# EmbodiedVision/diffsdfsim

Measured on AMD Instinct MI355X. Metric: sim steps/sec (fwd+bwd), 1024 batched 3D scenes x 8 SDF bodies, higher is better.
Workload: dtype f64

## Files before the change

### diffsdfsim_amd/csrc/contact_geom.h

```cpp
#pragma once
#include "geom.h"

namespace dss {
#if DSS_ALL_SHAPES
inline namespace shapes_all {
#else
inline namespace shapes_lean {
#endif

template <class T> struct BodyG {
    T q[4], pos[3];
    Shape<T> shape;
};

template <class T> __host__ __device__ inline double lap_probe(const Shape<T> &s, const T *p, double phi0, double h)
{
    Shape<double> sd;
    sd.type = s.type;
    for (int i = 0; i < 3; ++i) { sd.prm[i] = val(s.prm[i]); sd.hd[i] = val(s.hd[i]); }
    sd.scale = val(s.scale);
#if DSS_ALL_SHAPES
    sd.hr = val(s.hr);
    sd.lin = nullptr;
    sd.grid = s.grid;
    for (int i = 0; i < 3; ++i) sd.gn[i] = s.gn[i];
#endif
    double acc = 0.0, pt[3] = {val(p[0]), val(p[1]), val(p[2])}, g[3];
    for (int i = 0; i < 3; ++i) {
        double a, b, save = pt[i];
        pt[i] = save + h; query_sdf(sd, pt, a, g, false);
        pt[i] = save - h; query_sdf(sd, pt, b, g, false);
        pt[i] = save;
        acc += a - 2.0 * phi0 + b;
    }
    return acc;
}

template <class T>
__host__ __device__ inline void contact_head(const BodyG<T> &b1, const T tri[3][3], const double abc[3], T *cp1, T *n1, T &d1,
                                             T *p1)
{
    for (int i = 0; i < 3; ++i) cp1[i] = tri[0][i] * abc[0] + tri[1][i] * abc[1] + tri[2][i] * abc[2];
#if DSS_ALL_SHAPES
    if (b1.shape.type == SHAPE_IGR) {
        igr_lin(b1.shape, 0, cp1, d1, n1);
        for (int i = 0; i < 3; ++i) cp1[i] = cp1[i] - d1 * n1[i];
        igr_lin(b1.shape, 1, cp1, d1, n1);
        quat_apply(b1.q, cp1, p1);
        return;
    }
#endif
    query_sdf(b1.shape, cp1, d1, n1, true);
    for (int i = 0; i < 3; ++i) cp1[i] = cp1[i] - d1 * n1[i];
    query_sdf(b1.shape, cp1, d1, n1, true);
    quat_apply(b1.q, cp1, p1);
}
template <class T>
__host__ __device__ inline void contact_tail(const BodyG<T> &b1, const BodyG<T> &b2, const T *cp1, const T *n1, const T &d1,
                                             const T *p1, double lap_h, T *n, T *p2, T &pen, int *stable_io, bool detach_b2 = false)
{
    T cpw[3], rel[3], cp2[3], d2, n2[3], t[3];
    for (int i = 0; i < 3; ++i) { cpw[i] = p1[i] + b1.pos[i]; rel[i] = cpw[i] - b2.pos[i]; }
    quat_apply_inv(b2.q, rel, cp2);
    if (detach_b2) for (int i = 0; i < 3; ++i) cp2[i] = T(val(cp2[i]));
#if DSS_ALL_SHAPES
    if (b2.shape.type == SHAPE_IGR) igr_lin(b2.shape, 0, cp2, d2, n2);
    else
#endif
    query_sdf(b2.shape, cp2, d2, n2, true);
    bool stable;
    if (stable_io && *stable_io >= 0) stable = *stable_io != 0;
    else {
        const double l1 = lap_probe(b1.shape, cp1, val(d1), lap_h), l2 = lap_probe(b2.shape, cp2, val(d2), lap_h);
        stable = fabs(l2) < fabs(l1);
        if (stable_io) *stable_io = stable ? 1 : 0;
    }
    if (stable) {
        quat_apply(b2.q, n2, n);
    } else {
        quat_apply(b1.q, n1, t);
        for (int i = 0; i < 3; ++i) n[i] = -t[i];
    }
    for (int i = 0; i < 3; ++i) t[i] = cp2[i] - d2 * n2[i];
    quat_apply(b2.q, t, p2);
    pen = -d2;
}
template <class T>
__host__ __device__ inline void contact_from_bary(const BodyG<T> &b1, const BodyG<T> &b2, const T tri[3][3],
                                                  const double abc[3], double lap_h, T *n, T *p1, T *p2, T &pen,
                                                  int *stable_io = nullptr, bool detach_b2 = false)
{
    T cp1[3], n1[3], d1;
    contact_head(b1, tri, abc, cp1, n1, d1, p1);
    contact_tail(b1, b2, cp1, n1, d1, p1, lap_h, n, p2, pen, stable_io, detach_b2);
}

template <class T> __host__ __device__ inline T toc_D(const T *in)
{
    const T h = in[0], hc = in[1];
    const T *p1 = in + 2, *p2 = in + 5, *n = in + 8, *V1 = in + 11, *V2 = in + 17, *q1 = in + 23, *x1 = in + 27,
            *q2 = in + 30, *x2 = in + 34, *a1 = in + 37, *a2 = in + 40;
    T R1[9], R2[9], r1[9], r2[9], R10[9], R20[9], w[3], pos1[3], pos2[3];
    for (int i = 0; i < 3; ++i) { pos1[i] = x1[i] - hc * V1[3 + i]; pos2[i] = x2[i] - hc * V2[3 + i]; }
    for (int i = 0; i < 3; ++i) w[i] = -hc * V1[i];
    so3_exp(w, r1);
    for (int i = 0; i < 3; ++i) w[i] = -hc * V2[i];
    so3_exp(w, r2);
    quat_to_mat(q1, R1);
    quat_to_mat(q2, R2);
    for (int a = 0; a < 3; ++a)
        for (int b = 0; b < 3; ++b) {
            R10[3 * a + b] = r1[3 * a] * R1[b] + r1[3 * a + 1] * R1[3 + b] + r1[3 * a + 2] * R1[6 + b];
            R20[3 * a + b] = r2[3 * a] * R2[b] + r2[3 * a + 1] * R2[3 + b] + r2[3 * a + 2] * R2[6 + b];
        }
    T cs1[3], cs2[3], ns2[3];
    for (int i = 0; i < 3; ++i) {
        cs1[i] = R10[i] * p1[0] + R10[3 + i] * p1[1] + R10[6 + i] * p1[2];
        cs2[i] = R20[i] * p2[0] + R20[3 + i] * p2[1] + R20[6 + i] * p2[2];
        ns2[i] = R20[i] * n[0] + R20[3 + i] * n[1] + R20[6 + i] * n[2];
    }
    T dRi[9], dRj[9], Rih[9], Rjh[9];
    for (int i = 0; i < 3; ++i) w[i] = h * V1[i];
    so3_exp(w, dRi);
    for (int i = 0; i < 3; ++i) w[i] = h * V2[i];
    so3_exp(w, dRj);
    for (int a = 0; a < 3; ++a)
        for (int b = 0; b < 3; ++b) {
            Rih[3 * a + b] = dRi[3 * a] * R10[b] + dRi[3 * a + 1] * R10[3 + b] + dRi[3 * a + 2] * R10[6 + b];
            Rjh[3 * a + b] = dRj[3 * a] * R20[b] + dRj[3 * a + 1] * R20[3 + b] + dRj[3 * a + 2] * R20[6 + b];
        }
    T ciw[3], rel[3], D = T(0.0);
    for (int i = 0; i < 3; ++i) {
        const T pih = pos1[i] + h * V1[3 + i] + 0.5 * a1[i] * h * h, pjh = pos2[i] + h * V2[3 + i] + 0.5 * a2[i] * h * h;
        ciw[i] = Rih[3 * i] * cs1[0] + Rih[3 * i + 1] * cs1[1] + Rih[3 * i + 2] * cs1[2] + pih;
        rel[i] = ciw[i] - pjh;
    }
    for (int i = 0; i < 3; ++i) {
        const T cij = Rjh[i] * rel[0] + Rjh[3 + i] * rel[1] + Rjh[6 + i] * rel[2];
        D = D + ns2[i] * (cs2[i] - cij);
    }
    return D;
}

template <class T> __host__ __device__ inline void friction_dirs(const T *n, int nd, T D[][3])
{
    int am = 0;
    for (int i = 1; i < 3; ++i) if (fabs(val(n[i])) < fabs(val(n[am]))) am = i;
    T e[3] = {T(am == 0 ? 1.0 : 0.0), T(am == 1 ? 1.0 : 0.0), T(am == 2 ? 1.0 : 0.0)}, t[3];
    cross(e, n, t);
    normalize(t, D[0]);
    cross(D[0], n, t);
    normalize(t, D[1]);
    if (nd == 4) {
        for (int i = 0; i < 3; ++i) t[i] = D[0][i] + D[1][i];
        normalize(t, D[2]);
        cross(D[2], n, t);
        normalize(t, D[3]);
    }
}

}
}
```

### diffsdfsim_amd/csrc/narrowphase.hip

```cpp
#ifndef DSS_ALL_SHAPES
#define DSS_ALL_SHAPES 0
#endif
#if !DSS_ALL_SHAPES
#define DSS_STAMPS np
#endif

#include "launchers.h"
#include "np_common.h"

namespace {
constexpr int NP_WAVES = 3;
constexpr int OV_RUN = 256;
constexpr int OV_NT = 256;
__global__ void __launch_bounds__(OV_NT) overlap_kernel(DssWorld W)
{
    __shared__ unsigned char s_ok[64 * 63 / 2];
    __shared__ unsigned char s_big[64];
    const int nb = W.nb, nup = nb * (nb - 1) / 2, np = npairs_of(nb);
    const int sc = blockIdx.x, tid = threadIdx.x, lane = tid & 63, wv = tid >> 6;
    if (!W.active[sc]) return;
    const bool few = (long)W.B * np <= 256L * NP_WAVES;
    if (tid < nb) {
        const int nf = W.mesh_nf[W.mesh_id[(size_t)sc * nb + tid]];
        s_big[tid] = nf > WAVE_ITEM_MAX_FACES || (few && nf > 2048);
    }
#if DSS_ALL_SHAPES
    __shared__ unsigned char s_igr[64];
    if (tid < nb) s_igr[tid] = W.shape_type[(size_t)sc * nb + tid] == DSS_SHAPE_IGR;
#endif
    for (int up = wv; up < nup; up += OV_NT / 64) {
        int i = 0, rem = up;
        while (rem >= nb - 1 - i) { rem -= nb - 1 - i; ++i; }
        const int j = i + 1 + rem;
        int ok = !W.no_contact[i * nb + j];
        if (ok) {
            BodyD A, Bd;
            load_body(W, sc, i, A);
            load_body(W, sc, j, Bd);
            for (int dir = 0; dir < 2 && ok; ++dir) {
                const BodyD &src = dir ? Bd : A, &dst = dir ? A : Bd;
                const double s = dst.g.shape.scale;
                Region reg;
                region_of(src.g, dst.g, 1e-9, reg);
                const double *vbox = W.vch_box + (size_t)W.mesh_vch_off[src.mesh] * 6;
                const int nch = (src.nv + OV_RUN - 1) / OV_RUN;
                int found = 0;
                for (int cb0 = 0; cb0 < nch && !found; cb0 += 64) {
                    const int ch = cb0 + lane;
                    unsigned long long m = __ballot(ch < nch && box_hits(reg, vbox + (size_t)ch * 6));
                    while (m && !found) {
                        const int b = __ffsll((long long)m) - 1;
                        m &= m - 1;
                        int hit = 0;
#pragma unroll
                        for (int sub = 0; sub < OV_RUN / 64; ++sub) {
                            const int v = (cb0 + b) * OV_RUN + sub * 64 + lane;
                            if (v < src.nv) {
                                double p[3];
                                to_frame(src.g, dst.g, W.verts + (size_t)(src.voff + v) * 3, p);
                                hit |= (-s <= p[0] && p[0] <= s && -s <= p[1] && p[1] <= s && -s <= p[2] && p[2] <= s);
                            }
                        }
                        found = __ballot(hit) != 0ull;
                    }
                }
                ok = found;
            }
        }
        if (lane == 0) {
            s_ok[up] = (unsigned char)ok;
            W.ovl[((size_t)sc * nb + i) * nb + j] = ok;
            if (!ok) {
                W.pc_count[(size_t)sc * np + i * (nb - 1) + (j - 1)] = 0;
                W.pc_count[(size_t)sc * np + j * (nb - 1) + i] = 0;
            }
        }
    }
    __syncthreads();
    if (tid == 0) {
        int cnt[2] = {0, 0};
#if DSS_ALL_SHAPES
        int nig = 0;
        for (int up = 0, i = 0, j = 1; up < nup; ++up) {
            if (s_ok[up] && (s_igr[i] || s_igr[j])) nig += 2;
            if (++j == nb) { ++i; j = i + 1; }
        }
        if (nig) {
            int at = atomicAdd(W.n_pairs + 6, nig);
            for (int up = 0, i = 0, j = 1; up < nup; ++up) {
                if (s_ok[up] && (s_igr[i] || s_igr[j])) {
                    s_ok[up] = 0;
                    if (W.igr_list && at + 2 <= W.igr_items_cap) {
                        W.igr_list[at++] = sc * np + i * (nb - 1) + (j - 1);
                        W.igr_list[at++] = sc * np + j * (nb - 1) + i;
                    } else atomicOr(W.overflow + sc, 32);
                }
                if (++j == nb) { ++i; j = i + 1; }
            }
        }
#endif
        for (int up = 0, i = 0, j = 1; up < nup; ++up) {
            if (s_ok[up]) { ++cnt[s_big[i] ? 0 : 1]; ++cnt[s_big[j] ? 0 : 1]; }
            if (++j == nb) { ++i; j = i + 1; }
        }
        const int cap = W.B * np;
        const unsigned long long old = atomicAdd(reinterpret_cast<unsigned long long *>(W.n_pairs),
                                                 (unsigned long long)(unsigned)cnt[0] | ((unsigned long long)(unsigned)cnt[1] << 32));
        int at[2] = {(int)(old & 0xffffffffull), (int)(old >> 32)};
        for (int up = 0, i = 0, j = 1; up < nup; ++up) {
            if (s_ok[up]) {
                const int li = s_big[i] ? 0 : 1, lj = s_big[j] ? 0 : 1;
                W.pair_list[(size_t)li * cap + at[li]++] = sc * np + i * (nb - 1) + (j - 1);
                W.pair_list[(size_t)lj * cap + at[lj]++] = sc * np + j * (nb - 1) + i;
            }
            if (++j == nb) { ++i; j = i + 1; }
        }
    }
}

template <class G> __device__ int narrow_pair(const DssWorld &W, ScratchT<G> &S, int item, int slot_id)
{
    STAMP(0);
    item = dss_uniform(item); slot_id = dss_uniform(slot_id);
    const int np = npairs_of(W.nb);
    const int sc = item / np, dp = item % np, tid = G::tid();
    int a, b;
    pair_of(dp, W.nb, a, b);
    int *pc_count = W.pc_count + (size_t)sc * np + dp;
    BodyD A, Bd;
    load_body(W, sc, a, A);
    load_body(W, sc, b, Bd);
    const int MC = W.max_cand;
    int *__restrict__ cface = W.cand_face + (size_t)slot_id * 2 * MC, *__restrict__ kface = cface + MC;
    int *__restrict__ cstate = W.cand_state + (size_t)slot_id * MC;
    double *__restrict__ cb = W.cand_buf + (size_t)slot_id * DSS_CAND_FIELDS * MC;
    const double *__restrict__ m_verts = W.verts, *__restrict__ m_fcent = W.fcent;
    const int *__restrict__ m_faces = W.faces;
#define CB(f, k) cb[(size_t)(f) * MC + (k)]
    const double sB = Bd.g.shape.scale;

    double Ra[9], Rb[9], R12[9], t12[3];
    quat_to_mat(A.g.q, Ra);
    quat_to_mat(Bd.g.q, Rb);
    for (int i = 0; i < 3; ++i) {
        for (int j = 0; j < 3; ++j) R12[3 * i + j] = Rb[i] * Ra[j] + Rb[3 + i] * Ra[3 + j] + Rb[6 + i] * Ra[6 + j];
        t12[i] = Rb[i] * (A.g.pos[0] - Bd.g.pos[0]) + Rb[3 + i] * (A.g.pos[1] - Bd.g.pos[1]) + Rb[6 + i] * (A.g.pos[2] - Bd.g.pos[2]);
    }

    int ncand = 0, over = 0;
    Region reg;
    region_of(A.g, Bd.g, 1e-9, reg);
    const double *fbox = W.fch_box + (size_t)W.mesh_fch_off[A.mesh] * 6;
    constexpr int RUN = 256;
    const int nch = (A.nf + RUN - 1) / RUN, lane = tid & 63, wv = tid >> 6;
    auto cull_face = [&](const double *c) -> int {
        double cb2[3];
        for (int i = 0; i < 3; ++i) cb2[i] = R12[3 * i] * c[0] + R12[3 * i + 1] * c[1] + R12[3 * i + 2] * c[2] + t12[i];
        const double lim = sB + 1e-9 * (1.0 + sB);
        return fabs(cb2[0]) <= lim && fabs(cb2[1]) <= lim && fabs(cb2[2]) <= lim;
    };
    auto load_tri = [&](int f, double tri[3][3]) {
        const int *fv = m_faces + (size_t)(A.foff + f) * 3;
        for (int k = 0; k < 3; ++k) {
            const double *vp = m_verts + (size_t)(A.voff + fv[k]) * 3;
            for (int i = 0; i < 3; ++i) tri[k][i] = vp[i];
        }
    };
    auto test_tri = [&](double tri[3][3], double pqr[3][3]) -> int {
        double x[3] = {0, 0, 0};
        for (int k = 0; k < 3; ++k) {
            to_frame(A.g, Bd.g, tri[k], pqr[k]);
            for (int i = 0; i < 3; ++i) x[i] += pqr[k][i];
        }
        div3(x, 3.0, x);
        double phi, g[3], rad = 0.0;
        const bool box = Bd.g.shape.type == SHAPE_BOX;
        const bool in_cube = query_sdf(Bd.g.shape, x, phi, g, !box);
        for (int k = 0; k < 3; ++k) {
            const double d[3] = {x[0] - pqr[k][0], x[1] - pqr[k][1], x[2] - pqr[k][2]};
            const double r = t_sqrt(d[0] * d[0] + d[1] * d[1] + d[2] * d[2]);
            if (r > rad) rad = r;
        }
        if (box) return (phi < rad + W.eps) && in_cube;
        const double gn = t_sqrt(g[0] * g[0] + g[1] * g[1] + g[2] * g[2]);
        return (phi < rad + W.eps) && (gn > 1e-12);
    };
    auto full_face = [&](int f, double pqr[3][3]) -> int {
        double tri[3][3];
        load_tri(f, tri);
        return test_tri(tri, pqr);
    };
    auto test_face = [&](int f, double pqr[3][3]) -> int {
        return cull_face(m_fcent + (size_t)(A.foff + f) * 3) ? full_face(f, pqr) : 0;
    };
    if (G::BT == 64) {
        auto run_far = [&](const double *bx) -> bool {
#if DSS_ALL_SHAPES
            if (Bd.g.shape.type == SHAPE_GRID || Bd.g.shape.type == SHAPE_BOWL || Bd.g.shape.type == SHAPE_IGR) return false;
#endif
            double m[3], e2 = 0.0, emin = INFINITY;
            for (int i = 0; i < 3; ++i) {
                m[i] = 0.5 * (bx[i] + bx[3 + i]);
                const double e = 0.5 * (bx[3 + i] - bx[i]);
                e2 += e * e; emin = fmin(emin, e);
            }
            double pu[3], u, gdum[3];
            for (int i = 0; i < 3; ++i) pu[i] = (R12[3 * i] * m[0] + R12[3 * i + 1] * m[1] + R12[3 * i + 2] * m[2] + t12[i]) / sB;
            sdf_unit(Bd.g.shape, pu, u, gdum, false);
            return u * sB - sqrt(e2) >= emin + W.eps + 1e-9 * (1.0 + sB);
        };
        int npass = 0;
        for (int base = 0; base < nch; base += G::BT) {
            const int ch = base + tid;
            const int hit = ch < nch && box_hits(reg, fbox + (size_t)ch * 6) && !run_far(fbox + (size_t)ch * 6);
            const int slot = compact_slot(hit, npass, S);
            if (slot >= 0 && slot < G::HCAP) S.hidx[slot] = ch;
        }
        if (npass > G::HCAP) return 1;
        G::sync();
        int *surv = reinterpret_cast<int *>(S.hp);
        constexpr int SCAP = (int)(sizeof(S.hp) / sizeof(int)) - 4 * 64;
        int nsurv = 0;
        auto flush = [&]() {
            G::sync();
            for (int base = 0; base < nsurv; base += 128) {
                const int vA = base + lane < nsurv, vB = base + 64 + lane < nsurv;
                const int fA = vA ? surv[base + lane] : 0, fB = vB ? surv[base + 64 + lane] : 0;
                double triA[3][3], triB[3][3], pqr[3][3];
                load_tri(fA, triA);
                load_tri(fB, triB);
                const int flagA = test_tri(triA, pqr) && vA;
                const int slotA = compact_slot(flagA, ncand, S);
                if (slotA >= 0 && slotA < MC) {
                    cface[slotA] = fA;
                    for (int k = 0; k < 3; ++k) for (int i2 = 0; i2 < 3; ++i2) CB(3 * k + i2, slotA) = pqr[k][i2];
                }
                if (base + 64 >= nsurv) break;
                const int flagB = test_tri(triB, pqr) && vB;
                const int slotB = compact_slot(flagB, ncand, S);
                if (slotB >= 0 && slotB < MC) {
                    cface[slotB] = fB;
                    for (int k = 0; k < 3; ++k) for (int i2 = 0; i2 < 3; ++i2) CB(3 * k + i2, slotB) = pqr[k][i2];
                }
            }
            G::sync();
            nsurv = 0;
        };
        for (int i = 0; i < npass; ++i) {
            const int f0 = S.hidx[i] * RUN + lane;
            double c[4][3];
            for (int sub = 0; sub < 4; ++sub) {
                const int f = f0 + 64 * sub < A.nf ? f0 + 64 * sub : A.nf - 1;
                for (int d = 0; d < 3; ++d) c[sub][d] = m_fcent[(size_t)(A.foff + f) * 3 + d];
            }
            for (int sub = 0; sub < 4; ++sub) {
                const int ok = f0 + 64 * sub < A.nf && cull_face(c[sub]);
                const int slot = compact_slot(ok, nsurv, S);
                if (slot >= 0) surv[slot] = f0 + 64 * sub;
            }
            if (nsurv > SCAP) flush();
        }
        if (nsurv > 0) flush();
        if (ncand > MC) { over |= 1; ncand = MC; }
        if (tid == 0) { W.pc_stats[((size_t)sc * np + dp) * 2] = npass; W.pc_stats[((size_t)sc * np + dp) * 2 + 1] = ncand; }
        G::sync();
    } else if (nch <= G::CHCAP) {
        int npass = 0;
        for (int base = 0; base < nch; base += G::BT) {
            const int ch = base + tid;
            const int hit = ch < nch && box_hits(reg, fbox + (size_t)ch * 6);
            const int slot = compact_slot(hit, npass, S);
            if (slot >= 0) S.hidx[slot] = ch;
        }
        unsigned long long *words = reinterpret_cast<unsigned long long *>(S.hp);
        G::sync();
        for (int i = 0; i < npass; ++i)
            for (int sub = wv; sub < 4; sub += G::NW) {
                const int f = S.hidx[i] * RUN + sub * 64 + lane;
                double pqr[3][3];
                const int flag = f < A.nf ? test_face(f, pqr) : 0;
                const unsigned long long w = __ballot(flag);
                if (lane == 0) words[i * 4 + sub] = w;
            }
        G::sync();
        const int nw = npass * 4, per = (nw + G::BT - 1) / G::BT;
        int mine = 0;
        for (int e = tid * per; e < (tid + 1) * per && e < nw; ++e) mine += __popcll(words[e]);
        S.red_i[tid] = mine;
        G::sync();
        if (tid == 0) { int run = 0; for (int t = 0; t < G::BT; ++t) { const int v = S.red_i[t]; S.red_i[t] = run; run += v; } S.wave_tot[0] = run; }
        G::sync();
        ncand = S.wave_tot[0];
        {
            int run = S.red_i[tid];
            for (int e = tid * per; e < (tid + 1) * per && e < nw; ++e) { S.woff[e] = run; run += __popcll(words[e]); }
        }
        G::sync();
        if (ncand > 0)
            for (int i = 0; i < npass; ++i)
                for (int sub = wv; sub < 4; sub += G::NW) {
                    const unsigned long long w = words[i * 4 + sub];
                    if (!((w >> lane) & 1ull)) continue;
                    const int slot = S.woff[i * 4 + sub] + __popcll(w & ((1ull << lane) - 1ull));
                    if (slot >= MC) continue;
                    const int f = S.hidx[i] * RUN + sub * 64 + lane;
                    double pqr[3][3];
                    test_face(f, pqr);
                    cface[slot] = f;
                    for (int k = 0; k < 3; ++k) for (int i2 = 0; i2 < 3; ++i2) CB(3 * k + i2, slot) = pqr[k][i2];
                }
        if (ncand > MC) { over |= 1; ncand = MC; }
        if (tid == 0) { W.pc_stats[((size_t)sc * np + dp) * 2] = npass; W.pc_stats[((size_t)sc * np + dp) * 2 + 1] = ncand; }
        G::sync();
    } else {
        for (int base = 0; base < A.nf; base += G::BT) {
            if (!box_hits(reg, fbox + (size_t)(base / RUN) * 6)) continue;
            const int f = base + tid;
            double pqr[3][3];
            const int flag = f < A.nf ? test_face(f, pqr) : 0;
            if (!G::any(flag)) continue;
            const int slot = compact_slot(flag, ncand, S);
            if (slot >= 0 && slot < MC) {
                cface[slot] = f;
                for (int k = 0; k < 3; ++k) for (int i = 0; i < 3; ++i) CB(3 * k + i, slot) = pqr[k][i];
            }
            if (ncand > MC) { over |= 1; ncand = MC; }
        }
    }
    if (ncand == 0) { if (tid == 0) *pc_count = 0; return 0; }
    G::sync();
    STAMP(1);

    struct Cand { double pqr[9], x[3], abc[3]; };
    auto vtx = [](const Cand &c, int bi, int i) { return bi == 0 ? c.pqr[i] : (bi == 1 ? c.pqr[3 + i] : c.pqr[6 + i]); };
    auto load_c = [&](Cand &c, int k) {
        for (int i = 0; i < 9; ++i) c.pqr[i] = CB(i, k);
        for (int i = 0; i < 3; ++i) { c.x[i] = CB(9 + i, k); c.abc[i] = CB(12 + i, k); }
    };
    auto store_c = [&](const Cand &c, int k) {
        for (int i = 0; i < 3; ++i) { CB(9 + i, k) = c.x[i]; CB(12 + i, k) = c.abc[i]; }
    };
    auto init_c = [&](Cand &c) {
        double best = INFINITY; int bi = 0;
        for (int v = 0; v < 3; ++v) {
            double phi, g[3];
            query_sdf(Bd.g.shape, c.pqr + 3 * v, phi, g, false);
            if (phi < best) { best = phi; bi = v; }
        }
        for (int i = 0; i < 3; ++i) { c.x[i] = vtx(c, bi, i); c.abc[i] = (i == bi) ? 1.0 : 0.0; }
    };
    auto eval_c = [&](const Cand &c, int iter, float &gm, int &bi, int &pen) {
        double phi, g[3];
        query_sdf(Bd.g.shape, c.x, phi, g, true);
        double bestd = INFINITY; bi = 0;
        for (int v = 0; v < 3; ++v) {
            const double d = c.pqr[3 * v] * g[0] + c.pqr[3 * v + 1] * g[1] + c.pqr[3 * v + 2] * g[2];
            if (d < bestd) { bestd = d; bi = v; }
        }
        const double impr = (c.x[0] - vtx(c, bi, 0)) * g[0] + (c.x[1] - vtx(c, bi, 1)) * g[1] + (c.x[2] - vtx(c, bi, 2)) * g[2];
        gm = (fabs(impr) > W.tol) ? (float)(2.0 / (iter + 2.0)) : 0.0f;
        pen = phi < -W.tol;
    };
    auto apply_c = [&](Cand &c, float g32, int bi) {
        const double gm = (double)g32, om = (double)(1.0f - g32);
        for (int i = 0; i < 3; ++i) { c.x[i] = om * c.x[i] + gm * vtx(c, bi, i); c.abc[i] *= om; }
        for (int i = 0; i < 3; ++i) if (i == bi) c.abc[i] += gm;
    };
    int nmov = 0;
    {
        int vote = 0;
        for (int base = 0; base < ncand; base += G::BT) {
            const int k = base + tid;
            float gm = 0.0f; int bi = 0, pen = 0;
            if (k < ncand) {
                Cand c; load_c(c, k); init_c(c);
                eval_c(c, 0, gm, bi, pen);
                if (gm != 0.0f && !pen) apply_c(c, gm, bi);
                store_c(c, k);
                CB(25, k) = (double)gm; cstate[k] = bi;
            }
            const unsigned long long bm = __ballot(gm != 0.0f), bp = __ballot(pen);
            if ((tid & 63) == 0) S.vote[0][tid >> 6] = (bm != 0ull ? 1 : 0) | (bp != 0ull ? 2 : 0);
            G::sync();
            for (int w = 0; w < G::BT / 64; ++w) vote |= S.vote[0][w];
            const int slot = compact_slot(gm != 0.0f, nmov, S);
            if (slot >= 0 && slot < G::HCAP) S.hidx[slot] = k;
        }
        G::sync();
        if (vote & 2) {
            for (int k = tid; k < ncand; k += G::BT) {
                const float gm = (float)CB(25, k);
                if (gm != 0.0f) { Cand c; load_c(c, k); init_c(c); store_c(c, k); }
            }
            nmov = 0;
        }
        if (nmov > G::HCAP) { if (G::BT == 64) return 1; over |= 2; nmov = G::HCAP; }
        G::sync();
    }
    if (G::BT == 64 && nmov > 0 && nmov <= 16) {
        const int mi = tid >> 2, role = tid & 3, qbase = tid & ~3;
        Cand m0;
        const int k0 = mi < nmov ? S.hidx[mi] : -1;
        int alive = k0 >= 0;
        if (alive) load_c(m0, k0);
        for (int iter = 1; iter < 32; iter += 2) {
            Cand e = m0;
            if (role) apply_c(e, (float)(2.0 / (iter + 2.0)), role - 1);
            float gm = 0.0f; int bi = 0, pen = 0;
            if (alive) eval_c(e, role ? iter + 1 : iter, gm, bi, pen);
            const float gmA = __shfl(gm, qbase, 64);
            const int biA = __shfl(bi, qbase, 64), penA = __shfl(pen, qbase, 64);
            const unsigned long long bmA = __ballot(alive && gmA != 0.0f), bpA = __ballot(alive && penA);
            if (gmA == 0.0f) alive = 0;
            if (bmA == 0ull || bpA != 0ull) break;
            if (alive) apply_c(m0, gmA, biA);
            if (iter + 1 >= 32) break;
            const int src = qbase + 1 + biA;
            const float gmB = __shfl(gm, src, 64);
            const int biB = __shfl(bi, src, 64), penB = __shfl(pen, src, 64);
            const unsigned long long bmB = __ballot(alive && gmB != 0.0f), bpB = __ballot(alive && penB);
            if (gmB == 0.0f) alive = 0;
            if (bmB == 0ull || bpB != 0ull) break;
            if (alive) apply_c(m0, gmB, biB);
        }
        if (k0 >= 0 && role == 0) store_c(m0, k0);
        nmov = 0;
    }
    Cand m0;
    const int k0 = tid < nmov ? S.hidx[tid] : -1;
    int alive0 = k0 >= 0;
    if (alive0) load_c(m0, k0);
    for (int iter = 1; iter < 32 && nmov > 0; ++iter) {
        float gam[MAX_CPT]; int ind[MAX_CPT];
        int any_pen = 0, moving = 0, q = 1, pen;
        gam[0] = 0.0f; ind[0] = 0;
        if (alive0) {
            eval_c(m0, iter, gam[0], ind[0], pen);
            any_pen |= pen; moving |= gam[0] != 0.0f;
            if (gam[0] == 0.0f) alive0 = 0;
        }
        for (int j = tid + G::BT; j < nmov; j += G::BT, ++q) {
            const int k = S.hidx[j];
            gam[q] = 0.0f; ind[q] = 0;
            if (cstate[k] < 0) continue;
            Cand c; load_c(c, k);
            eval_c(c, iter, gam[q], ind[q], pen);
            any_pen |= pen; moving |= gam[q] != 0.0f;
            if (gam[q] == 0.0f) cstate[k] = -1;
        }
        const unsigned long long bm = __ballot(moving), bp = __ballot(any_pen);
        if ((tid & 63) == 0) S.vote[iter & 1][tid >> 6] = (bm != 0ull ? 1 : 0) | (bp != 0ull ? 2 : 0);
        G::sync();
        int vote = 0;
        for (int w = 0; w < G::BT / 64; ++w) vote |= S.vote[iter & 1][w];
        if (!(vote & 1) || (vote & 2)) break;
        if (gam[0] != 0.0f) apply_c(m0, gam[0], ind[0]);
        q = 1;
        for (int j = tid + G::BT; j < nmov; j += G::BT, ++q) {
            if (gam[q] == 0.0f) continue;
            const int k = S.hidx[j];
            Cand c; load_c(c, k); apply_c(c, gam[q], ind[q]); store_c(c, k);
        }
    }
    if (k0 >= 0) store_c(m0, k0);
    G::sync();

    STAMP(2);
    double qrel[4];
    {
        double qbi[4];
        quat_inv(Bd.g.q, qbi);
        quat_mul(qbi, A.g.q, qrel);
    }
    int ncon = 0, bad = 0;
    for (int base = 0; base < ncand; base += G::BT) {
        const int k = base + tid;
        int flag = 0, kf = 0;
        double abc[3] = {0, 0, 0}, n[3] = {0, 0, 0}, p1[3] = {0, 0, 0}, p2[3] = {0, 0, 0}, pen = 0.0;
        if (k < ncand) {
            const int f = cface[k];
            const int *fv = m_faces + (size_t)(A.foff + f) * 3;
            double tri[3][3], xb1[3] = {0, 0, 0};
            for (int v = 0; v < 3; ++v) {
                abc[v] = CB(12 + v, k);
                const double *vp = m_verts + (size_t)(A.voff + fv[v]) * 3;
                for (int i = 0; i < 3; ++i) { tri[v][i] = vp[i]; xb1[i] += tri[v][i] * abc[v]; }
            }
            double phi1, g1[3], gr[3], x[3], phi2, g2[3];
            query_sdf(A.g.shape, xb1, phi1, g1, true);
            quat_apply(qrel, g1, gr);
            for (int i = 0; i < 3; ++i) x[i] = CB(9 + i, k) - phi1 * gr[i];
            query_sdf(Bd.g.shape, x, phi2, g2, false);
            flag = phi2 <= W.eps;
            if (flag) {
                int stable = -1;
                contact_from_bary(A.g, Bd.g, tri, abc, 1e-3, n, p1, p2, pen, &stable);
                kf = stable ? f : (f | DSS_FACE_NORMAL1);
                if (!(pen <= W.tol)) bad = 1;
            }
        }
        if (!G::any(flag)) continue;
        const int slot = compact_slot(flag, ncon, S);
        if (slot >= 0) {
            kface[slot] = kf;
            for (int i = 0; i < 3; ++i) {
                CB(15 + i, slot) = abc[i]; CB(18 + i, slot) = n[i]; CB(21 + i, slot) = p1[i]; CB(i, slot) = p2[i];
            }
            CB(24, slot) = pen;
            if (slot < G::HCAP) S.cst[slot] = t_sqrt(n[0] * n[0] + n[1] * n[1] + n[2] * n[2]) > 1e-12 ? 0 : 255;
        }
    }
    if (ncon == 0) { if (tid == 0) { *pc_count = 0; if (over) atomicOr(W.overflow + sc, over); } return 0; }
    G::sync();

    STAMP(3);
    if (G::any(bad)) {
        if (tid == 0) { W.invalid[sc] = 1; *pc_count = 0; }
        if (!W.strict_no_pen && W.dt_try[sc] > 0.0 && W.dt_try[sc] < W.dt / 1024.0) { G::sync(); emit_unfiltered<G>(W, sc, dp, ncon, over, kface, cb, MC); }
        return 0;
    }

#define NP_PRESTATE 1
#include "np_filter_emit.inc"
#undef NP_PRESTATE
#undef CB
}

union NpScratch {
    ScratchT<BlockGroup> blk;
    ScratchT<WaveGroup> wav[BlockGroup::NW];
};
template <bool DEFERRED> __global__ void __launch_bounds__(NT, NP_WAVES) narrowphase_kernel(DssWorld W_arg)
{
    DSS_KERNARG_REF(DssWorld, W, W_arg);
    __shared__ NpScratch S;
    __shared__ int s_item;
    const int cap = W.B * npairs_of(W.nb), seg = DEFERRED ? 2 : 0;
    {
        const int n = W.n_pairs[DEFERRED ? 4 : 0];
        const int *list = W.pair_list + (size_t)seg * cap;
        for (;;) {
            __syncthreads();
            if (threadIdx.x == 0) s_item = atomicAdd(W.n_pairs + (DEFERRED ? 5 : 2), 1);
            __syncthreads();
            const int it = s_item;
            if (it >= n) break;
            narrow_pair<BlockGroup>(W, S.blk, list[it], (int)blockIdx.x * BlockGroup::NW);
        }
    }
    if (DEFERRED) return;
    __syncthreads();
    const int n = W.n_pairs[1], lane = threadIdx.x & 63;
    const int *list = W.pair_list + cap;
    ScratchT<WaveGroup> &Sw = S.wav[threadIdx.x >> 6];
    for (;;) {
        int it = 0;
        if (lane == 0) it = atomicAdd(W.n_pairs + 3, 1);
        it = __shfl(it, 0);
        if (it >= n) break;
        const int item = list[it];
        if (narrow_pair<WaveGroup>(W, Sw, item, (int)(blockIdx.x * BlockGroup::NW + (threadIdx.x >> 6))) && lane == 0)
            W.pair_list[(size_t)2 * cap + atomicAdd(W.n_pairs + 4, 1)] = item;
        dss_wave_sync();
    }
}

__global__ void __launch_bounds__(64) compact_contacts_kernel(DssWorld W, int *nc_out, int *body_out, int *face_out,
                                                               double *abc_out, double *geom_out)
{
    constexpr int MAXSLOT = 64 * 63;
    __shared__ int s_off[MAXSLOT + 1];
    __shared__ short s_a[MAXSLOT], s_b[MAXSLOT];
    __shared__ unsigned char s_neg[MAXSLOT];
    const int sc = blockIdx.x, lane = threadIdx.x, nb = W.nb, np = npairs_of(nb), MP = W.max_pc, MX = W.maxc;
    if (!W.active[sc]) return;
    int run = 0;
    for (int base = 0; base < np; base += 64) {
        const int slot = base + lane;
        int cnt = 0, a = 0, b = 0;
        if (slot < np) {
            int i = 0, rem = slot >> 1;
            while (rem >= nb - 1 - i) { rem -= nb - 1 - i; ++i; }
            const int j = i + 1 + rem;
            a = (slot & 1) ? j : i; b = (slot & 1) ? i : j;
            cnt = W.pc_count[(size_t)sc * np + a * (nb - 1) + (b < a ? b : b - 1)];
        }
        const int fwd = __shfl_up(cnt, 1, 64);
        if ((slot & 1) && fwd < 0) cnt = 0;
        if (slot < np) s_neg[slot] = cnt < 0;
        if (cnt < 0) cnt = -cnt;
        int incl = cnt;
        for (int d = 1; d < 64; d <<= 1) { const int o = __shfl_up(incl, d, 64); if (lane >= d) incl += o; }
        if (slot < np) { s_off[slot] = run + incl - cnt; s_a[slot] = (short)a; s_b[slot] = (short)b; }
        run += __shfl(incl, 63, 64);
    }
    if (lane == 0) s_off[np] = run;
    __syncthreads();
    const int total = run < MX ? run : MX;
    for (int o = lane; o < total; o += 64) {
        int lo = 0, hi = np;
        while (hi - lo > 1) { const int mid = (lo + hi) >> 1; if (s_off[mid] <= o) lo = mid; else hi = mid; }
        const int a = s_a[lo], b = s_b[lo], k = o - s_off[lo];
        const size_t dp = (size_t)sc * np + a * (nb - 1) + (b < a ? b : b - 1);
        const int *pf = W.pc_face + dp * MP;
        const double *pabc = W.pc_abc + dp * 3 * MP, *pg = W.pc_geom + dp * 10 * MP;
        const int face = s_neg[lo] ? -1 - pf[k] : pf[k];
        double abc[3], geo[10];
        for (int f = 0; f < 3; ++f) abc[f] = pabc[(size_t)f * MP + k];
        for (int f = 0; f < 10; ++f) geo[f] = pg[(size_t)f * MP + k];
        body_out[(size_t)sc * 2 * MX + o] = a;
        body_out[(size_t)sc * 2 * MX + MX + o] = b;
        face_out[(size_t)sc * MX + o] = face;
        for (int f = 0; f < 3; ++f) abc_out[((size_t)sc * 3 + f) * MX + o] = abc[f];
        for (int f = 0; f < 10; ++f) geom_out[((size_t)sc * 10 + f) * MX + o] = geo[f];
    }
    if (lane == 0) {
        if (run > MX) atomicOr(W.overflow + sc, 8);
        nc_out[sc] = total;
    }
}

}

namespace dss {
static inline int np_grid(int B, int nb)
{
    const long items = (long)B * nb * (nb - 1);
    return (int)(items < 256 * NP_WAVES ? items : 256 * NP_WAVES);
}
#if DSS_ALL_SHAPES
int launch_find_contacts_all(const DssWorld &W, int *nc_out, int *body_out, int *face_out, double *abc_out,
                             double *geom_out, hipStream_t stream)
{
#else
int launch_find_contacts(const DssWorld &W, int *nc_out, int *body_out, int *face_out, double *abc_out,
                         double *geom_out, hipStream_t stream)
{
    if (W.shape_rare) return launch_find_contacts_all(W, nc_out, body_out, face_out, abc_out, geom_out, stream);
#endif
    static_assert(BlockGroup::HCAP <= BlockGroup::BT * MAX_CPT && WaveGroup::HCAP <= WaveGroup::BT * MAX_CPT, "mover registers");
    if (W.max_cand < 1 || W.nb < 1) return DSS_E_UNSUPPORTED;
    if (W.nb < 2) {
        hipLaunchKernelGGL(compact_contacts_kernel, dim3(W.B), dim3(64), 0, stream, W, nc_out, body_out, face_out, abc_out, geom_out);
        return hipGetLastError() == hipSuccess ? DSS_OK : DSS_E_UNSUPPORTED;
    }
    const int nup = W.nb * (W.nb - 1) / 2, np = W.nb * (W.nb - 1);
    (void)hipMemsetAsync(W.n_pairs, 0, 8 * sizeof(int), stream);
    hipLaunchKernelGGL(overlap_kernel, dim3(W.B), dim3(OV_NT), 0, stream, W);
    const int grid = np_grid(W.B, W.nb);
    hipLaunchKernelGGL(narrowphase_kernel<false>, dim3(grid), dim3(NT), 0, stream, W);
    hipLaunchKernelGGL(narrowphase_kernel<true>, dim3(grid < 64 ? grid : 64), dim3(NT), 0, stream, W);
#if DSS_ALL_SHAPES
    if (W.igr_list) { const int rc = launch_igr_rounds(W, stream); if (rc) return rc; }
#endif
    hipLaunchKernelGGL(compact_contacts_kernel, dim3(W.B), dim3(64), 0, stream, W, nc_out, body_out, face_out, abc_out, geom_out);
    return hipGetLastError() == hipSuccess ? DSS_OK : DSS_E_UNSUPPORTED;
}
}

#if !DSS_ALL_SHAPES
extern "C" int dss_np_slots(int B, int nb) { return dss::np_grid(B, nb) * 4; }
#endif
```

### diffsdfsim_amd/csrc/np_filter_emit.inc

```
    STAMP(4);
    int nkeep = 0;
    unsigned keptbits = 0u;
    if (ncon <= 1) {
        if (tid == 0) cstate[0] = -2;
        nkeep = ncon;
    } else {
        const bool lds_state = ncon <= G::HCAP;
        if (!lds_state && G::BT == 64) return 1;
        auto get_state = [&](int k) -> int { return lds_state ? (int)S.cst[k] : cstate[k]; };
        auto set_state = [&](int k, int v) { if (lds_state) S.cst[k] = (unsigned char)v; else cstate[k] = v; };
#if defined(NP_PRESTATE)
        if (!lds_state)
#endif
        for (int k = tid; k < ncon; k += G::BT) {
            const double nn = t_sqrt(CB(18, k) * CB(18, k) + CB(19, k) * CB(19, k) + CB(20, k) * CB(20, k));
            set_state(k, nn > 1e-12 ? 0 : 255);
        }
        G::sync();
        for (int cl = 1; cl <= ncon; ++cl) {
            int mine = -1;
            for (int k = tid; k < ncon; k += G::BT) if (get_state(k) == 0) { mine = k; break; }
            const int seed = block_argmin(mine >= 0 ? (double)mine : INFINITY, mine, S);
            if (seed < 0) break;
            const double sn[3] = {CB(18, seed), CB(19, seed), CB(20, seed)};
            int m = 0;
            for (int base = 0; base < ncon; base += G::BT) {
                const int k = base + tid;
                int in = 0;
                double p1v[3] = {0.0, 0.0, 0.0};
                if (k < ncon && get_state(k) == 0) {
                    const double nk[3] = {CB(18, k), CB(19, k), CB(20, k)};
                    for (int i = 0; i < 3; ++i) p1v[i] = CB(21 + i, k);
                    const double d = fmin(nk[0] * sn[0] + nk[1] * sn[1] + nk[2] * sn[2], 1.0);
                    constexpr double C01 = 0.99995000041666528;
                    in = d > C01 + 1e-12 ? 1 : (d < C01 - 1e-12 ? 0 : (int)(acos(d) < 1e-2));
                }
#if DSS_ALL_SHAPES
                const int slot = compact_slot(in, m, S);
                if (slot >= 0) {
                    set_state(k, 3);
                    if (slot < G::HCAP) { S.hidx[slot] = k; for (int i = 0; i < 3; ++i) S.hp[3 * slot + i] = p1v[i]; }
                }
            }
            G::sync();
            if (m <= G::HCAP) {
                if (cluster_hull(S, HullLds<G>{&S}, m, W.eps)) return 1;
                for (int j = tid; j < m; j += G::BT) set_state(S.hidx[j], S.hflag[j] ? 2 : 1);
            } else {
                if (G::BT == 64) return 1;
                m = 0;
                for (int base = 0; base < ncon; base += G::BT) {
                    const int k = base + tid;
                    const int in = k < ncon && get_state(k) == 3;
                    const int slot = compact_slot(in, m, S);
                    if (slot >= 0) { cface[slot] = k; for (int i = 0; i < 3; ++i) CB(3 + i, slot) = CB(21 + i, k); }
                }
                G::sync();
                const HullGlobal P{cb, MC};
                cluster_hull(S, P, m, W.eps);
                for (int j = tid; j < m; j += G::BT) set_state(cface[j], P.getf(j) ? 2 : 1);
            }
            G::sync();
        }
#else
                const int slot = compact_slot(in, m, S);
                if (slot >= 0) {
                    set_state(k, 1);
                    if (slot < G::HCAP) { S.hidx[slot] = k; for (int i = 0; i < 3; ++i) S.hp[3 * slot + i] = p1v[i]; }
                }
            }
            G::sync();
            if (m > G::HCAP) { if (G::BT == 64) return 1; over |= 2; m = G::HCAP; }
            if (cluster_hull(S, HullLds<G>{&S}, m, W.eps) == 2) over |= 128;
            for (int j = tid; j < m; j += G::BT) if (S.hflag[j]) set_state(S.hidx[j], 2);
            G::sync();
        }
#endif
        for (int k = tid, r = 0; k < ncon; k += G::BT, ++r) {
            const int kept = get_state(k) == 2;
#if DSS_ALL_SHAPES
            if (r < 32)
#endif
            keptbits |= (unsigned)kept << r;
            nkeep += kept;
        }
        nkeep = (int)(block_sum((double)nkeep, S) + 0.5);
    }

    STAMP(5);
    int nout = 0;
    const int MP = W.max_pc;
    int *pf = W.pc_face + ((size_t)sc * np + dp) * MP;
    double *pabc = W.pc_abc + ((size_t)sc * np + dp) * 3 * MP, *pg = W.pc_geom + ((size_t)sc * np + dp) * 10 * MP;
    if (ncon <= 1) {
        if (tid == 0) {
            pf[0] = kface[0];
            for (int i = 0; i < 3; ++i) { pabc[(size_t)i * MP] = CB(15 + i, 0); pg[(size_t)i * MP] = CB(18 + i, 0); pg[(size_t)(3 + i) * MP] = CB(21 + i, 0); pg[(size_t)(6 + i) * MP] = CB(i, 0); }
            pg[(size_t)9 * MP] = CB(24, 0);
        }
        nout = 1;
    } else {
        for (int base = 0, r = 0; base < ncon; base += G::BT, ++r) {
            const int k = base + tid;
#if DSS_ALL_SHAPES
            const int flag = (k < ncon) && (r < 32 ? (int)((keptbits >> r) & 1u) : (cstate[k] == 2));
#else
            const int flag = (k < ncon) && ((keptbits >> r) & 1u);
#endif
            if (!G::any(flag)) continue;
            const int slot = compact_slot(flag, nout, S);
            if (slot >= 0 && slot < MP) {
                pf[slot] = kface[k];
                for (int i = 0; i < 3; ++i) {
                    pabc[(size_t)i * MP + slot] = CB(15 + i, k);
                    pg[(size_t)i * MP + slot] = CB(18 + i, k); pg[(size_t)(3 + i) * MP + slot] = CB(21 + i, k); pg[(size_t)(6 + i) * MP + slot] = CB(i, k);
                }
                pg[(size_t)9 * MP + slot] = CB(24, k);
            }
        }
        if (nout > MP) { over |= 4; nout = MP; }
    }
    if (tid == 0) { *pc_count = nout; if (over) atomicOr(W.overflow + sc, over); }
    STAMP(6);
    return 0;
```

Before: 516.3.

## Defer Laplacian normal-stability probes until clustering needs them

Contact generation now computes both candidate normals per contact and skips the costly Laplacian stability probe, which does 12 extra SDF queries. Probes run lazily only for the first block of contacts, for cluster seeds, for contacts whose cluster membership would differ between the two normals, and for finally kept contacts. This cuts SDF evaluations in the narrowphase but adds extra syncs, compaction passes and stored columns, and relies on the fallback being exact to preserve results.

```diff
diff --git a/diffsdfsim_amd/csrc/contact_geom.h b/diffsdfsim_amd/csrc/contact_geom.h
--- a/diffsdfsim_amd/csrc/contact_geom.h
+++ b/diffsdfsim_amd/csrc/contact_geom.h
@@ -35,6 +35,13 @@
     }
     return acc;
 }
+template <class T>
+__host__ __device__ inline bool contact_normal_stable(const Shape<T> &s1, const T *cp1, const T &d1, const Shape<T> &s2,
+                                                      const T *cp2, const T &d2, double lap_h)
+{
+    const double l1 = lap_probe(s1, cp1, val(d1), lap_h), l2 = lap_probe(s2, cp2, val(d2), lap_h);
+    return fabs(l2) < fabs(l1);
+}
 
 template <class T>
 __host__ __device__ inline void contact_head(const BodyG<T> &b1, const T tri[3][3], const double abc[3], T *cp1, T *n1, T &d1,
@@ -55,6 +62,27 @@
     query_sdf(b1.shape, cp1, d1, n1, true);
     quat_apply(b1.q, cp1, p1);
 }
+template <class T> __host__ __device__ inline void contact_head_pull(const BodyG<T> &b1, T *cp1, T *n1, T &d1, T *p1)
+{
+    for (int i = 0; i < 3; ++i) cp1[i] = cp1[i] - d1 * n1[i];
+    query_sdf(b1.shape, cp1, d1, n1, true);
+    quat_apply(b1.q, cp1, p1);
+}
+template <class T>
+__host__ __device__ inline void contact_tail_both(const BodyG<T> &b1, const BodyG<T> &b2, const T *n1, const T *p1, T *nA, T *nB,
+                                                  T *p2, T &pen, T *cp2)
+{
+    T cpw[3], rel[3], d2, n2[3], t[3];
+    for (int i = 0; i < 3; ++i) { cpw[i] = p1[i] + b1.pos[i]; rel[i] = cpw[i] - b2.pos[i]; }
+    quat_apply_inv(b2.q, rel, cp2);
+    query_sdf(b2.shape, cp2, d2, n2, true);
+    quat_apply(b2.q, n2, nB);
+    quat_apply(b1.q, n1, t);
+    for (int i = 0; i < 3; ++i) nA[i] = -t[i];
+    for (int i = 0; i < 3; ++i) t[i] = cp2[i] - d2 * n2[i];
+    quat_apply(b2.q, t, p2);
+    pen = -d2;
+}
 template <class T>
 __host__ __device__ inline void contact_tail(const BodyG<T> &b1, const BodyG<T> &b2, const T *cp1, const T *n1, const T &d1,
                                              const T *p1, double lap_h, T *n, T *p2, T &pen, int *stable_io, bool detach_b2 = false)
@@ -71,8 +99,7 @@
     bool stable;
     if (stable_io && *stable_io >= 0) stable = *stable_io != 0;
     else {
-        const double l1 = lap_probe(b1.shape, cp1, val(d1), lap_h), l2 = lap_probe(b2.shape, cp2, val(d2), lap_h);
-        stable = fabs(l2) < fabs(l1);
+        stable = contact_normal_stable(b1.shape, cp1, d1, b2.shape, cp2, d2, lap_h);
         if (stable_io) *stable_io = stable ? 1 : 0;
     }
     if (stable) {
diff --git a/diffsdfsim_amd/csrc/narrowphase.hip b/diffsdfsim_amd/csrc/narrowphase.hip
--- a/diffsdfsim_amd/csrc/narrowphase.hip
+++ b/diffsdfsim_amd/csrc/narrowphase.hip
@@ -7,6 +7,10 @@
 
 #include "launchers.h"
 #include "np_common.h"
+
+#if !DSS_ALL_SHAPES
+#define NP_LAZY 1
+#endif
 
 namespace {
 constexpr int NP_WAVES = 3;
@@ -118,6 +122,34 @@
     }
 }
 
+#if defined(NP_LAZY)
+constexpr int NP_RESOLVED = 16;
+template <class G>
+__device__ __noinline__ void resolve_normals(const DssWorld &W, int sc, int a, int b, double *__restrict__ cb, int MC,
+                                             int *__restrict__ kface, unsigned char *cst, const int *list, int n)
+{
+    Shape<double> s[2];
+    for (int j = 0; j < 2; ++j) {
+        const size_t bi = (size_t)sc * W.nb + (j ? b : a);
+        make_shape(s[j], W.shape_type[bi], W.shape_prm + bi * 3);
+        for (int i = 0; i < 3; ++i) { s[j].prm[i] = dss_uniform(s[j].prm[i]); s[j].hd[i] = dss_uniform(s[j].hd[i]); }
+        s[j].scale = dss_uniform(s[j].scale);
+        s[j].type = dss_uniform(s[j].type);
+    }
+    for (int j = G::tid(); j < n; j += G::BT) {
+        const int k = list ? list[j] : j;
+        double cp1[3], cp2[3];
+        for (int i = 0; i < 3; ++i) { cp1[i] = cb[(size_t)(6 + i) * MC + k]; cp2[i] = cb[(size_t)(9 + i) * MC + k]; }
+        const double d1 = cb[(size_t)12 * MC + k], d2 = -cb[(size_t)24 * MC + k];
+        if (!contact_normal_stable(s[0], cp1, d1, s[1], cp2, d2, 1e-3)) {
+            for (int i = 0; i < 3; ++i) cb[(size_t)(18 + i) * MC + k] = cb[(size_t)(3 + i) * MC + k];
+            kface[k] |= DSS_FACE_NORMAL1;
+        }
+        if (cst) cst[k] |= NP_RESOLVED;
+    }
+}
+#endif
+
 template <class G> __device__ int narrow_pair(const DssWorld &W, ScratchT<G> &S, int item, int slot_id)
 {
     STAMP(0);
@@ -473,10 +505,40 @@
         quat_mul(qbi, A.g.q, qrel);
     }
     int ncon = 0, bad = 0;
+#if defined(NP_LAZY)
+    int ambu = 0;
+#endif
     for (int base = 0; base < ncand; base += G::BT) {
         const int k = base + tid;
         int flag = 0, kf = 0;
         double abc[3] = {0, 0, 0}, n[3] = {0, 0, 0}, p1[3] = {0, 0, 0}, p2[3] = {0, 0, 0}, pen = 0.0;
+#if defined(NP_LAZY)
+        double nA[3] = {0, 0, 0}, cp1[3] = {0, 0, 0}, cp2[3] = {0, 0, 0}, d1 = 0.0;
+        if (k < ncand) {
+            const int f = cface[k];
+            const int *fv = m_faces + (size_t)(A.foff + f) * 3;
+            double tri[3][3];
+            for (int v = 0; v < 3; ++v) {
+                abc[v] = CB(12 + v, k);
+                const double *vp = m_verts + (size_t)(A.voff + fv[v]) * 3;
+                for (int i = 0; i < 3; ++i) tri[v][i] = vp[i];
+            }
+            for (int i = 0; i < 3; ++i) cp1[i] = tri[0][i] * abc[0] + tri[1][i] * abc[1] + tri[2][i] * abc[2];
+            double n1[3], gr[3], x[3], phi2, g2[3];
+            query_sdf(A.g.shape, cp1, d1, n1, true);
+            quat_apply(qrel, n1, gr);
+            for (int i = 0; i < 3; ++i) x[i] = CB(9 + i, k) - d1 * gr[i];
+            query_sdf(Bd.g.shape, x, phi2, g2, false);
+            flag = phi2 <= W.eps;
+            if (flag) {
+                contact_head_pull(A.g, cp1, n1, d1, p1);
+                contact_tail_both(A.g, Bd.g, n1, p1, nA, n, p2, pen, cp2);
+                kf = f;
+                if (!(pen <= W.tol)) bad = 1;
+                if ((t_sqrt(nA[0] * nA[0] + nA[1] * nA[1] + nA[2] * nA[2]) > 1e-12) != (t_sqrt(n[0] * n[0] + n[1] * n[1] + n[2] * n[2]) > 1e-12)) ambu = 1;
+            }
+        }
+#else
         if (k < ncand) {
             const int f = cface[k];
             const int *fv = m_faces + (size_t)(A.foff + f) * 3;
@@ -499,6 +561,7 @@
                 if (!(pen <= W.tol)) bad = 1;
             }
         }
+#endif
         if (!G::any(flag)) continue;
         const int slot = compact_slot(flag, ncon, S);
         if (slot >= 0) {
@@ -507,7 +570,13 @@
                 CB(15 + i, slot) = abc[i]; CB(18 + i, slot) = n[i]; CB(21 + i, slot) = p1[i]; CB(i, slot) = p2[i];
             }
             CB(24, slot) = pen;
+#if defined(NP_LAZY)
+            for (int i = 0; i < 3; ++i) { CB(3 + i, slot) = nA[i]; CB(6 + i, slot) = cp1[i]; CB(9 + i, slot) = cp2[i]; }
+            CB(12, slot) = d1;
+            if (slot < G::HCAP) S.cst[slot] = t_sqrt(n[0] * n[0] + n[1] * n[1] + n[2] * n[2]) > 1e-12 ? 0 : 8;
+#else
             if (slot < G::HCAP) S.cst[slot] = t_sqrt(n[0] * n[0] + n[1] * n[1] + n[2] * n[2]) > 1e-12 ? 0 : 255;
+#endif
         }
     }
     if (ncon == 0) { if (tid == 0) { *pc_count = 0; if (over) atomicOr(W.overflow + sc, over); } return 0; }
@@ -516,7 +585,14 @@
     STAMP(3);
     if (G::any(bad)) {
         if (tid == 0) { W.invalid[sc] = 1; *pc_count = 0; }
-        if (!W.strict_no_pen && W.dt_try[sc] > 0.0 && W.dt_try[sc] < W.dt / 1024.0) { G::sync(); emit_unfiltered<G>(W, sc, dp, ncon, over, kface, cb, MC); }
+        if (!W.strict_no_pen && W.dt_try[sc] > 0.0 && W.dt_try[sc] < W.dt / 1024.0) {
+            G::sync();
+#if defined(NP_LAZY)
+            resolve_normals<G>(W, sc, a, b, cb, MC, kface, nullptr, nullptr, ncon);
+            G::sync();
+#endif
+            emit_unfiltered<G>(W, sc, dp, ncon, over, kface, cb, MC);
+        }
         return 0;
     }
 
diff --git a/diffsdfsim_amd/csrc/np_filter_emit.inc b/diffsdfsim_amd/csrc/np_filter_emit.inc
--- a/diffsdfsim_amd/csrc/np_filter_emit.inc
+++ b/diffsdfsim_amd/csrc/np_filter_emit.inc
@@ -1,20 +1,45 @@
     STAMP(4);
     int nkeep = 0;
     unsigned keptbits = 0u;
+#if defined(NP_LAZY)
+    constexpr int NONORMAL = 8;
+#else
+    constexpr int NONORMAL = 255;
+#endif
     if (ncon <= 1) {
+#if defined(NP_LAZY)
+        resolve_normals<G>(W, sc, a, b, cb, MC, kface, nullptr, nullptr, ncon);
+        G::sync();
+#endif
         if (tid == 0) cstate[0] = -2;
         nkeep = ncon;
     } else {
         const bool lds_state = ncon <= G::HCAP;
         if (!lds_state && G::BT == 64) return 1;
+#if defined(NP_LAZY)
+        const bool amb_any = G::any(ambu);
+        const bool lazy = lds_state && ncon > G::BT && !amb_any;
+        resolve_normals<G>(W, sc, a, b, cb, MC, kface, lazy ? S.cst : nullptr, nullptr, lazy ? G::BT : ncon);
+        G::sync();
+        auto get_state = [&](int k) -> int { return lds_state ? (int)(S.cst[k] & 15) : cstate[k]; };
+        auto set_state = [&](int k, int v) { if (lds_state) S.cst[k] = (unsigned char)((S.cst[k] & NP_RESOLVED) | v); else cstate[k] = v; };
+        auto resolve_listed = [&](const int *list, int n) {
+            G::sync();
+            resolve_normals<G>(W, sc, a, b, cb, MC, kface, S.cst, list, n);
+            G::sync();
+        };
+#else
         auto get_state = [&](int k) -> int { return lds_state ? (int)S.cst[k] : cstate[k]; };
         auto set_state = [&](int k, int v) { if (lds_state) S.cst[k] = (unsigned char)v; else cstate[k] = v; };
-#if defined(NP_PRESTATE)
+#endif
+#if defined(NP_LAZY)
+        if (!lds_state || amb_any)
+#elif defined(NP_PRESTATE)
         if (!lds_state)
 #endif
         for (int k = tid; k < ncon; k += G::BT) {
             const double nn = t_sqrt(CB(18, k) * CB(18, k) + CB(19, k) * CB(19, k) + CB(20, k) * CB(20, k));
-            set_state(k, nn > 1e-12 ? 0 : 255);
+            set_state(k, nn > 1e-12 ? 0 : NONORMAL);
         }
         G::sync();
         for (int cl = 1; cl <= ncon; ++cl) {
@@ -22,19 +47,42 @@
             for (int k = tid; k < ncon; k += G::BT) if (get_state(k) == 0) { mine = k; break; }
             const int seed = block_argmin(mine >= 0 ? (double)mine : INFINITY, mine, S);
             if (seed < 0) break;
+#if defined(NP_LAZY)
+            if (lazy && !(S.cst[seed] & NP_RESOLVED)) {
+                if (tid == 0) S.red_i[0] = seed;
+                resolve_listed(S.red_i, 1);
+            }
+#endif
             const double sn[3] = {CB(18, seed), CB(19, seed), CB(20, seed)};
+            auto member = [&](double n0, double n1, double n2) -> int {
+                const double d = fmin(n0 * sn[0] + n1 * sn[1] + n2 * sn[2], 1.0);
+                constexpr double C01 = 0.99995000041666528;
+                return d > C01 + 1e-12 ? 1 : (d < C01 - 1e-12 ? 0 : (int)(acos(d) < 1e-2));
+            };
             int m = 0;
             for (int base = 0; base < ncon; base += G::BT) {
                 const int k = base + tid;
                 int in = 0;
                 double p1v[3] = {0.0, 0.0, 0.0};
+#if defined(NP_LAZY)
+                int open = 0;
+#endif
                 if (k < ncon && get_state(k) == 0) {
-                    const double nk[3] = {CB(18, k), CB(19, k), CB(20, k)};
                     for (int i = 0; i < 3; ++i) p1v[i] = CB(21 + i, k);
-                    const double d = fmin(nk[0] * sn[0] + nk[1] * sn[1] + nk[2] * sn[2], 1.0);
-                    constexpr double C01 = 0.99995000041666528;
-                    in = d > C01 + 1e-12 ? 1 : (d < C01 - 1e-12 ? 0 : (int)(acos(d) < 1e-2));
+                    in = member(CB(18, k), CB(19, k), CB(20, k));
+#if defined(NP_LAZY)
+                    if (lazy && !(S.cst[k] & NP_RESOLVED)) open = member(CB(3, k), CB(4, k), CB(5, k)) != in;
+#endif
                 }
+#if defined(NP_LAZY)
+                if (lazy && G::any(open)) {
+                    int nopen = 0;
+                    const int at = compact_slot(open, nopen, S);
+                    if (at >= 0) S.red_i[at] = k;
+                    resolve_listed(S.red_i, nopen);
+                    if (open) in = member(CB(18, k), CB(19, k), CB(20, k));
+                }
+#endif
 #if DSS_ALL_SHAPES
                 const int slot = compact_slot(in, m, S);
                 if (slot >= 0) {
@@ -85,6 +133,17 @@
             nkeep += kept;
         }
         nkeep = (int)(block_sum((double)nkeep, S) + 0.5);
+#if defined(NP_LAZY)
+        if (lazy) {
+            int nopen = 0;
+            for (int base = 0; base < ncon; base += G::BT) {
+                const int k = base + tid;
+                const int at = compact_slot(k < ncon && S.cst[k] == 2, nopen, S);
+                if (at >= 0) S.hidx[at] = k;
+            }
+            resolve_listed(S.hidx, nopen);
+        }
+#endif
     }
 
     STAMP(5);
```

New measurement: 484.7. -6.1%, worse.
